# TopJohn/corda

Measured on AMD Instinct MI355X. Metric: signature verifications/sec (whole node, 1/2/4/8 GPU) + % integer-ALU peak, higher is better.
Workload: dtype u32

## Files before the change

### corda_amd/csrc/ed25519.hip

```cpp
#ifndef FE_QUAD
#define FE_QUAD 0
#endif
#ifndef FE_USE_ASM2
#define FE_USE_ASM2 1
#endif
#include <hip/hip_runtime.h>

#include <functional>
#include <stdint.h>
#include <stdlib.h>

#include "ed25519_ops.hpp"
#include "ed25519_route.hpp"
#include "ed25519_ws.hpp"
#include "sha2_device.hpp"
#include "status.hpp"

namespace cordahip {

__global__ void __launch_bounds__(64) ed25519_btable_kernel(uint32_t* __restrict__ tab) {
  const int g = blockIdx.x * blockDim.x + threadIdx.x;
  if (g >= 2 * kBTableEntries) return;
  const int k = g % kBTableEntries;
  ge_p3 B, P;
  ge_base(B);
  if (g >= kBTableEntries)
    for (int t = 0; t < kBDigits * kBBits; t++) ge_dbl<true>(B, B);
  ge_cached bc;
  ge_to_cached(bc, B);
  ge_identity(P);
  for (int bit = kBBits - 1; bit >= 0; bit--) {
    ge_dbl<true>(P, P);
    if ((k >> bit) & 1) ge_add<true>(P, P, bc);
  }
  store_niels_entry(tab + g * kBEntryWords, P);
  if (g == 0) {
    ge_cached id;
    fe_set(id.YpX, 1);
    fe_set(id.YmX, 1);
    fe_set(id.Z, 1);
    fe_set(id.T2d, 0);
    store_cached(tab + kBIdentityWord, id);
  }
}

CDEV bool mp8_ge(const uint32_t a[8], const uint32_t b[8]) {
  uint32_t br = 0;
#pragma unroll
  for (int i = 0; i < 8; i++) br = (uint32_t)(((uint64_t)a[i] - b[i] - br) >> 63);
  return br == 0;
}
CDEV void mp8_add(uint32_t r[8], const uint32_t a[8], const uint32_t b[8]) {
  uint64_t c = 0;
#pragma unroll
  for (int i = 0; i < 8; i++) {
    c += (uint64_t)a[i] + b[i];
    r[i] = (uint32_t)c;
    c >>= 32;
  }
}
CDEV void mp8_neg(uint32_t a[8]) {
  uint64_t c = 1;
#pragma unroll
  for (int i = 0; i < 8; i++) {
    c += (uint64_t)(~a[i]);
    a[i] = (uint32_t)c;
    c >>= 32;
  }
}
CDEV void mp8_copy(uint32_t d[8], const uint32_t s[8]) {
#pragma unroll
  for (int i = 0; i < 8; i++) d[i] = s[i];
}
CDEV int mp8_absbits(const uint32_t a[8]) {
  uint32_t t[8];
  mp8_copy(t, a);
  if (a[7] >> 31) mp8_neg(t);
  return mp8_bitlen(t);
}

CDEV double mp8_f64(const uint32_t a[8]) {
  double d = (double)a[7];
#pragma unroll
  for (int i = 6; i >= 0; i--) d = fma(d, 4294967296.0, (double)a[i]);
  return d;
}
CDEV void mp8_submul(uint32_t a[8], const uint32_t b[8], uint32_t q) {
  uint64_t pc = 0;
  uint32_t br = 0;
#pragma unroll
  for (int i = 0; i < 8; i++) {
    const uint64_t p = (uint64_t)q * b[i] + pc;
    pc = p >> 32;
    const uint64_t d = (uint64_t)a[i] - (uint32_t)p - br;
    a[i] = (uint32_t)d;
    br = (uint32_t)(d >> 63);
  }
}
CDEV void mp8_shl_dyn(uint32_t o[8], const uint32_t b[8], int k) {
  const int ws = k >> 5, bs = k & 31;
#pragma unroll
  for (int i = 0; i < 8; i++) {
    const uint32_t lo = (i - ws >= 0) ? word_sel(b, i - ws) : 0u;
    const uint32_t lo2 = (i - ws - 1 >= 0) ? word_sel(b, i - ws - 1) : 0u;
    o[i] = bs ? ((lo << bs) | (lo2 >> (32 - bs))) : lo;
  }
}

CDEV void euclid_divstep(uint32_t rp[8], const uint32_t rc[8], uint32_t tp[8], const uint32_t tc[8]) {
  const double inv = 1.0 / mp8_f64(rc);
  while (mp8_ge(rp, rc)) {
    const double qd = mp8_f64(rp) * inv * (1.0 - 0x1p-40);
    if (qd < 4294967296.0) {
      uint32_t q = (uint32_t)qd;
      q = q ? q : 1u;
      mp8_submul(rp, rc, q);
      mp8_submul(tp, tc, q);
    } else {
      const int e = (int)((__double_as_longlong(qd) >> 52) & 0x7ff) - 1023;
      const int k = e - 31;
      const uint32_t q = (uint32_t)(qd * __longlong_as_double((long long)(1023 - k) << 52));
      uint32_t bs[8], ts[8];
      mp8_shl_dyn(bs, rc, k);
      mp8_shl_dyn(ts, tc, k);
      mp8_submul(rp, bs, q);
      mp8_submul(tp, ts, q);
    }
  }
}

CDEV double mp8_top(const uint32_t a[8], int s) {
  const int w = s >> 5, b = s & 31;
  const uint64_t lo = ((uint64_t)word_sel(a, w + 1) << 32) | word_sel(a, w);
  const uint64_t hi = word_sel(a, w + 2);
  return (double)((lo >> b) | (b ? hi << (64 - b) : 0ull));
}
CDEV void mp8_lincomb(uint32_t o[8], const uint32_t x[8], int a, const uint32_t y[8], int b) {
  const uint32_t ua = (uint32_t)(a < 0 ? -a : a), ub = (uint32_t)(b < 0 ? -b : b);
  uint64_t pc = 0, qc = 0;
  uint32_t br = 0;
#pragma unroll
  for (int i = 0; i < 8; i++) {
    const uint64_t p = (uint64_t)ua * x[i] + pc;
    pc = p >> 32;
    const uint64_t q = (uint64_t)ub * y[i] + qc;
    qc = q >> 32;
    const uint64_t d = (uint64_t)(uint32_t)p - (uint32_t)q - br;
    o[i] = (uint32_t)d;
    br = (uint32_t)(d >> 63);
  }
  if (b > 0 || (b == 0 && a < 0)) mp8_neg(o);
}

CDEV void half_scalars(uint32_t c0abs[8], bool& c0neg, uint32_t c1[8], const uint32_t h[8]) {
  const uint32_t kM[8] = {0xe7ae9f68u, 0xc09318d2u, 0x17bce6b2u, 0xa6f7cef5u, 0u, 0u, 0u, 0x80000000u};
  const uint32_t kS[8] = {0x754abea0u, 0x597d89b3u, 0xf9de6484u, 0xb504f333u, 0u, 0u, 0u, 0u};
  uint32_t rp[8], rc[8], tp[8], tc[8];
#pragma unroll
  for (int i = 0; i < 8; i++) {
    rp[i] = kM[i];
    rc[i] = h[i];
    tp[i] = 0;
    tc[i] = i == 0;
  }
  for (;;) {
    const int s = max(mp8_bitlen(rp) - 52, 0);
    double uh = mp8_top(rp, s), vh = mp8_top(rc, s);
    const double th = mp8_top(kS, s) + 1.0;
    double A = 1.0, B = 0.0, C = 0.0, D = 1.0;
    int n = 0;
    for (;;) {
      const double d1 = vh + C, d2 = vh + D;
      if (!(d1 > 0.0 && d2 > 0.0)) break;
      const double n1 = uh + A;
      double q = floor(n1 / d1);
      const double r1 = fma(-q, d1, n1);
      q = r1 < 0.0 ? q - 1.0 : (r1 >= d1 ? q + 1.0 : q);
      const double r2 = fma(-q, d2, uh + B);
      if (!(r2 >= 0.0 && r2 < d2)) break;
      const double nC = fma(-q, C, A), nD = fma(-q, D, B), nv = fma(-q, vh, uh);
      const double mc = fmax(fabs(nC), fabs(nD));
      if (nv - mc < th || mc >= 0x1p30) break;
      A = C;
      B = D;
      C = nC;
      D = nD;
      uh = vh;
      vh = nv;
      n++;
    }
    if (n == 0) break;
    const int a = (int)A, b = (int)B, c = (int)C, d = (int)D;
    uint32_t x[8], y[8];
    mp8_lincomb(x, rp, a, rc, b);
    mp8_lincomb(y, rp, c, rc, d);
    mp8_copy(rp, x);
    mp8_copy(rc, y);
    mp8_lincomb(x, tp, a, tc, b);
    mp8_lincomb(y, tp, c, tc, d);
    mp8_copy(tp, x);
    mp8_copy(tc, y);
  }
  while (mp8_ge(rc, kS)) {
    euclid_divstep(rp, rc, tp, tc);
#pragma unroll
    for (int i = 0; i < 8; i++) {
      const uint32_t a = rp[i], b = tp[i];
      rp[i] = rc[i];
      rc[i] = a;
      tp[i] = tc[i];
      tc[i] = b;
    }
  }
  uint32_t a0[8], a1[8];
  mp8_copy(a0, rc);
  mp8_copy(a1, tc);
  if (!(tc[0] & 1)) {
    uint32_t r3[8], t3[8];
    mp8_copy(r3, rp);
    mp8_copy(t3, tp);
    euclid_divstep(r3, rc, t3, tc);
    uint32_t p0[8], p1[8], m0[8], m1[8], nr3[8], nt3[8];
    mp8_add(p0, rc, r3);
    mp8_add(p1, tc, t3);
    mp8_copy(nr3, r3);
    mp8_neg(nr3);
    mp8_copy(nt3, t3);
    mp8_neg(nt3);
    mp8_add(m0, rc, nr3);
    mp8_add(m1, tc, nt3);
    int best = max(mp8_absbits(r3), mp8_absbits(t3));
    mp8_copy(a0, r3);
    mp8_copy(a1, t3);
    const int bp = max(mp8_absbits(p0), mp8_absbits(p1));
    if (bp < best) {
      best = bp;
      mp8_copy(a0, p0);
      mp8_copy(a1, p1);
    }
    const int bm = max(mp8_absbits(m0), mp8_absbits(m1));
    if (bm < best) {
      mp8_copy(a0, m0);
      mp8_copy(a1, m1);
    }
  }
  if (a1[7] >> 31) {
    mp8_neg(a0);
    mp8_neg(a1);
  }
  c0neg = (a0[7] >> 31) != 0;
  if (c0neg) mp8_neg(a0);
  mp8_copy(c0abs, a0);
  mp8_copy(c1, a1);
}

CDEV bool ge_strict_ok(const ge_p3& R, const uint32_t w[8]) {
  uint32_t all_ones = (w[7] & 0x7fffffffu) == 0x7fffffffu;
#pragma unroll
  for (int i = 1; i < 7; i++) all_ones &= (w[i] == 0xffffffffu);
  if (all_ones && w[0] >= 0xffffffedu) return false;
  return !((w[7] >> 31) && fe_iszero(R.X));
}

CDEV void store_point(uint32_t* __restrict__ o, const ge_p3& p) {
  uint4* o4 = reinterpret_cast<uint4*>(o);
  uint32_t w[32];
#pragma unroll
  for (int i = 0; i < 10; i++) {
    w[i] = p.X.v[i];
    w[10 + i] = p.Y.v[i];
    w[20 + i] = p.T.v[i];
  }
  w[30] = w[31] = 0;
#pragma unroll
  for (int q = 0; q < 8; q++) o4[q] = make_uint4(w[4 * q], w[4 * q + 1], w[4 * q + 2], w[4 * q + 3]);
}
CDEV void load_point(ge_p3& p, const uint32_t* __restrict__ o) {
  const uint4* o4 = reinterpret_cast<const uint4*>(o);
  uint32_t w[32];
#pragma unroll
  for (int q = 0; q < 8; q++) {
    const uint4 v = o4[q];
    w[4 * q] = v.x;
    w[4 * q + 1] = v.y;
    w[4 * q + 2] = v.z;
    w[4 * q + 3] = v.w;
  }
#pragma unroll
  for (int i = 0; i < 10; i++) {
    p.X.v[i] = w[i];
    p.Y.v[i] = w[10 + i];
    p.T.v[i] = w[20 + i];
  }
  fe_set(p.Z, 1);
}

#ifndef ED_PREP_LDS
#define ED_PREP_LDS 1
#endif
#if !ED_PREP_LDS
static constexpr int kParkP = joint_index(2, 2), kParkQ = joint_index(2, -2);
#endif
static constexpr int kPqT2d = 30, kPqQ = 40, kPqWords = 70;

CDEV uint32_t* joint_slot(uint32_t* rec, int idx) { return rec + kWhTab + idx * kWhEntryWords; }

CDEV void pq_store(uint32_t* col, int at, const fe& f) {
#pragma unroll
  for (int i = 0; i < 10; i++) col[(at + i) * 256] = f.v[i];
}
CDEV void pq_load(fe& f, const uint32_t* col, int at) {
#pragma unroll
  for (int i = 0; i < 10; i++) f.v[i] = col[(at + i) * 256];
}

CDEV void load_cached_niels(ge_niels& n, const uint32_t* __restrict__ p) {
  ge_cached c;
  load_cached(c, p);
  n.ypx = c.YpX;
  n.ymx = c.YmX;
  n.xy2d = c.T2d;
}

CDEV void park_point(uint32_t* __restrict__ rec, uint32_t* col, int which, const ge_p3& p) {
#if ED_PREP_LDS
  pq_store(col, which * kPqQ, p.X);
  pq_store(col, which * kPqQ + 10, p.Y);
  pq_store(col, which * kPqQ + 20, p.T);
#else
  store_point(joint_slot(rec, which ? kParkQ : kParkP), p);
#endif
}
CDEV void load_parked(ge_p3& p, uint32_t* __restrict__ rec, const uint32_t* col, int which) {
#if ED_PREP_LDS
  pq_load(p.X, col, which * kPqQ);
  pq_load(p.Y, col, which * kPqQ + 10);
  pq_load(p.T, col, which * kPqQ + 20);
  fe_set(p.Z, 1);
#else
  load_point(p, joint_slot(rec, which ? kParkQ : kParkP));
#endif
}
CDEV void park_niels(uint32_t* col, int pass, const ge_cached& c) {
#if ED_PREP_LDS
  if (pass) {
    pq_store(col, kPqQ, c.YpX);
    pq_store(col, kPqQ + 10, c.YmX);
    pq_store(col, kPqQ + 20, c.T2d);
  } else {
    pq_store(col, kPqT2d, c.T2d);
  }
#endif
}
CDEV void load_parked_niels(ge_niels& n, uint32_t* __restrict__ rec, const uint32_t* col, int which) {
#if ED_PREP_LDS
  if (which) {
    pq_load(n.ypx, col, kPqQ);
    pq_load(n.ymx, col, kPqQ + 10);
    pq_load(n.xy2d, col, kPqQ + 20);
  } else {
    fe x, y;
    pq_load(x, col, 0);
    pq_load(y, col, 10);
    fe_add(n.ypx, y, x);
    fe_sub(n.ymx, y, x);
    pq_load(n.xy2d, col, kPqT2d);
  }
#else
  load_cached_niels(n, joint_slot(rec, which ? joint_index(0, 1) : joint_index(1, 0)));
#endif
}

CDEV void joint_single_pass(uint32_t* __restrict__ rec, uint32_t* col, int pass) {
  ge_p3 B, D;
  load_parked(B, rec, col, pass);
  ge_cached c;
  ge_to_cached(c, B);
  park_niels(col, pass, c);
  store_cached(joint_slot(rec, pass ? joint_index(0, 1) : joint_index(1, 0)), c);
  ge_dbl<true>(D, B);
  ge_to_cached(c, D);
  store_cached(joint_slot(rec, pass ? joint_index(0, 2) : joint_index(2, 0)), c);
}

CDEV void joint_sign_pass(uint32_t* __restrict__ rec, uint32_t* col, int s) {
  ge_p3 D, E;
  ge_niels nq, np;
  ge_cached c;
  load_parked(D, rec, col, 0);
  load_parked_niels(nq, rec, col, 1);
  niels_cneg(nq, s < 0);
  ge_madd<true>(D, D, nq);
  ge_to_cached(c, D);
  store_cached(joint_slot(rec, joint_index(1, s)), c);
  ge_madd<true>(E, D, nq);
  ge_to_cached(c, E);
  store_cached(joint_slot(rec, joint_index(1, 2 * s)), c);
#if ED_PREP_LDS
  PHASE_BARRIER();
#endif
  load_parked_niels(np, rec, col, 0);
  ge_madd<true>(E, D, np);
  ge_to_cached(c, E);
  store_cached(joint_slot(rec, joint_index(2, s)), c);
  ge_dbl<true>(E, D);
  ge_to_cached(c, E);
  store_cached(joint_slot(rec, joint_index(2, 2 * s)), c);
}


#ifndef ED_PREP_WAVES
#define ED_PREP_WAVES 2
#endif
CDEV uint8_t prep_decode_phase(const uint8_t* __restrict__ keys, const uint8_t* __restrict__ sigs, uint64_t i,
                               uint32_t msg_len, const uint8_t* __restrict__ pre_status, uint32_t empty_is_error,
                               uint32_t* __restrict__ rec, uint32_t* col, uint32_t abyte[8], uint32_t Rw[8]) {
  uint8_t st = kStatusPending;
  load8(Rw, reinterpret_cast<const uint32_t*>(sigs + i * 64));
  {
    uint32_t wa[8];
    load8(wa, reinterpret_cast<const uint32_t*>(keys + i * 32));
    ge_p3 A, R;
    bool okA, okR;
    ge_frombytes_i2p_pair(A, okA, wa, R, okR, Rw);
    if (!okA) st = kStatusBadKey;
    else if (pre_status && pre_status[i] != kStatusOk) st = pre_status[i];
    else if (msg_len == 0 && empty_is_error) st = kStatusEmpty;
    fe_tobytes(abyte, A.Y);
    abyte[7] |= fe_isnegative(A.X) << 31;
    if (st == kStatusPending && !(okR && ge_strict_ok(R, Rw))) st = kStatusBadSig;
    if (st != kStatusPending) {
      ge_identity(A);
      ge_identity(R);
    }
    fe_neg(A.X, A.X);
    fe_neg(A.T, A.T);
    fe_neg(R.X, R.X);
    fe_neg(R.T, R.T);
    park_point(rec, col, 0, A);
    park_point(rec, col, 1, R);
  }
  return st;
}

CDEV void prep_table_phase(uint32_t* __restrict__ rec, uint32_t* col) {
#pragma unroll 1
  for (int pass = 0; pass < 2; pass++) {
    joint_single_pass(rec, col, pass);
    PHASE_BARRIER();
  }
#pragma unroll 1
  for (int s = -1; s <= 1; s += 2) {
    joint_sign_pass(rec, col, s);
    PHASE_BARRIER();
  }
}

CDEV uint8_t prep_keys_phase(const uint8_t* __restrict__ keys, const uint8_t* __restrict__ sigs, uint64_t i,
                             uint32_t msg_len, const uint8_t* __restrict__ pre_status, uint32_t empty_is_error,
                             uint32_t* __restrict__ rec, uint32_t* col, uint32_t abyte[8], uint32_t Rw[8]) {
  const uint8_t st = prep_decode_phase(keys, sigs, i, msg_len, pre_status, empty_is_error, rec, col, abyte, Rw);
  PHASE_BARRIER();
  prep_table_phase(rec, col);
  return st;
}

CDEV void prep_msg_phase(const uint8_t* __restrict__ sigs, const uint8_t* __restrict__ msgs, uint32_t msg_len,
                         uint64_t i, uint8_t st, const uint32_t abyte[8], const uint32_t Rw[8],
                         uint32_t* __restrict__ rec) {
  uint32_t ka[8], kr[8], e[8];
  bool c0neg = false;
  if (st == kStatusPending) {
    uint32_t S[8], hd[16], h[8], se[8], zero[8];
    load8(S, reinterpret_cast<const uint32_t*>(sigs + i * 64 + 32));
    sha512_segments(hd, Rw, abyte, true, msgs + i * (uint64_t)msg_len, msg_len);
    sc_reduce512(h, hd);
    sc_effective_S(se, S, slide_drops_carry(S));
    half_scalars(ka, c0neg, kr, h);
#pragma unroll
    for (int q = 0; q < 8; q++) zero[q] = 0;
    sc_muladd(e, kr, se, zero);
  } else {
#pragma unroll
    for (int q = 0; q < 8; q++) ka[q] = kr[q] = e[q] = 0;
  }
#if ED_SEL_STREAM
  uint32_t sel[32];
  sel_recode(sel, ka, kr, e, c0neg);
  sel[kSelWords] = 0;
  uint4* o4 = reinterpret_cast<uint4*>(rec + kWhSel);
#pragma unroll
  for (int q = 0; q < 8; q++) o4[q] = make_uint4(sel[4 * q], sel[4 * q + 1], sel[4 * q + 2], sel[4 * q + 3]);
#else
  store8(rec + kWhKa, ka);
  store8(rec + kWhKr, kr);
  store8(rec + kWhE, e);
  reinterpret_cast<uint4*>(rec + kWhFlags)[0] = make_uint4(c0neg ? 1u : 0u, 0u, 0u, 0u);
#endif
}

#if ED_PREP_LDS
#define PREP_PARK_COLUMN(col)                  \
  __shared__ uint32_t pq_lds[kPqWords][256]; \
  uint32_t* col = &pq_lds[0][threadIdx.x]
#else
#define PREP_PARK_COLUMN(col) uint32_t* col = nullptr
#endif

__global__ void __launch_bounds__(256) __attribute__((amdgpu_waves_per_eu(ED_PREP_WAVES))) ed25519_prep_half_kernel(
    const uint8_t* __restrict__ keys, const uint8_t* __restrict__ sigs, const uint8_t* __restrict__ msgs,
    uint32_t msg_len, uint64_t base, uint64_t m, const uint8_t* __restrict__ pre_status,
    uint8_t* __restrict__ status, uint32_t* __restrict__ ws, uint32_t empty_is_error) {
  const uint64_t li = (uint64_t)blockIdx.x * blockDim.x + threadIdx.x;
  if (li >= m) return;
  const uint64_t i = base + li;
  uint32_t* rec = ws + li * kWhLaneWords;
  uint32_t abyte[8], Rw[8];
  PREP_PARK_COLUMN(col);
  const uint8_t st = prep_keys_phase(keys, sigs, i, msg_len, pre_status, empty_is_error, rec, col, abyte, Rw);
  prep_msg_phase(sigs, msgs, msg_len, i, st, abyte, Rw, rec);
  status[i] = st;
}

__global__ void __launch_bounds__(256) __attribute__((amdgpu_waves_per_eu(ED_PREP_WAVES)))
ed25519_prep_half_idx_kernel(const uint8_t* __restrict__ keys, const uint8_t* __restrict__ sigs,
                             const uint8_t* __restrict__ msgs, uint32_t msg_len, uint64_t base, uint64_t m,
                             const uint8_t* __restrict__ pre_status, uint8_t* __restrict__ status,
                             uint32_t* __restrict__ ws, uint32_t empty_is_error, const uint32_t* __restrict__ scratch,
                             uint64_t lanes) {
  const uint64_t li = (uint64_t)blockIdx.x * blockDim.x + threadIdx.x;
  if (li >= route_chunk_lanes(scratch[kRouteCntGeneric], base, m)) return;
  const uint64_t i = scratch[route_off_generic(lanes) + base + li];
  uint32_t* rec = ws + li * kWhLaneWords;
  uint32_t abyte[8], Rw[8];
  PREP_PARK_COLUMN(col);
  const uint8_t st = prep_keys_phase(keys, sigs, i, msg_len, pre_status, empty_is_error, rec, col, abyte, Rw);
  prep_msg_phase(sigs, msgs, msg_len, i, st, abyte, Rw, rec);
  status[i] = st;
}

__global__ void __launch_bounds__(256) __attribute__((amdgpu_waves_per_eu(ED_PREP_WAVES))) ed25519_prep_keys_kernel(
    const uint8_t* __restrict__ keys, const uint8_t* __restrict__ sigs, uint32_t msg_len, uint64_t base, uint64_t m,
    const uint8_t* __restrict__ pre_status, uint8_t* __restrict__ status, uint32_t* __restrict__ ws,
    uint32_t empty_is_error) {
  const uint64_t li = (uint64_t)blockIdx.x * blockDim.x + threadIdx.x;
  if (li >= m) return;
  const uint64_t i = base + li;
  uint32_t* rec = ws + li * kWhLaneWords;
  uint32_t abyte[8], Rw[8];
  PREP_PARK_COLUMN(col);
  status[i] = prep_keys_phase(keys, sigs, i, msg_len, pre_status, empty_is_error, rec, col, abyte, Rw);
  store8(rec + kWhKa, abyte);
}

__global__ void __launch_bounds__(256) __attribute__((amdgpu_waves_per_eu(ED_PREP_WAVES))) ed25519_prep_msg_kernel(const uint8_t* __restrict__ sigs,
                                                               const uint8_t* __restrict__ msgs, uint32_t msg_len,
                                                               uint64_t base, uint64_t m,
                                                               const uint8_t* __restrict__ status,
                                                               uint32_t* __restrict__ ws) {
  const uint64_t li = (uint64_t)blockIdx.x * blockDim.x + threadIdx.x;
  if (li >= m) return;
  const uint64_t i = base + li;
  uint32_t* rec = ws + li * kWhLaneWords;
  uint32_t abyte[8], Rw[8];
  load8(abyte, rec + kWhKa);
  load8(Rw, reinterpret_cast<const uint32_t*>(sigs + i * 64));
  prep_msg_phase(sigs, msgs, msg_len, i, status[i], abyte, Rw, rec);
}

CDEV void fixed_base_mult(ge_p3& P, const uint32_t k[8], const uint32_t* __restrict__ btab) {
  ge_identity(P);
  for (int j = 31; j >= 0; j--) {
    if (j != 31) {
#pragma unroll
      for (int t = 0; t < 7; t++) ge_dbl<false>(P, P);
      ge_dbl<true>(P, P);
    }
    const int d = booth_digit<8>(k, j);
    ge_niels nb;
    load_niels(nb, btab, d < 0 ? -d : d);
    niels_cneg(nb, d < 0);
    ge_madd<true>(P, P, nb);
  }
}

__global__ void __launch_bounds__(256) ed25519_sign_kernel(const uint8_t* __restrict__ seeds,
                                                          const uint8_t* __restrict__ msgs, uint32_t msg_len,
                                                          uint64_t n, const uint32_t* __restrict__ btab,
                                                          uint8_t* __restrict__ pubs, uint8_t* __restrict__ sigs) {
  const uint64_t i = (uint64_t)blockIdx.x * blockDim.x + threadIdx.x;
  if (i >= n) return;
  uint32_t seed[8];
  {
    const uint4* s4 = reinterpret_cast<const uint4*>(seeds + i * 32);
    const uint4 a = s4[0], b = s4[1];
    seed[0] = a.x; seed[1] = a.y; seed[2] = a.z; seed[3] = a.w;
    seed[4] = b.x; seed[5] = b.y; seed[6] = b.z; seed[7] = b.w;
  }
  const uint8_t* msg = msgs + i * (uint64_t)msg_len;
  uint32_t hs[16], dummy[8];
#pragma unroll
  for (int q = 0; q < 8; q++) dummy[q] = 0;
  sha512_segments(hs, seed, dummy, false, msg, 0);
  uint32_t a[8], prefix[8];
#pragma unroll
  for (int q = 0; q < 8; q++) {
    a[q] = hs[q];
    prefix[q] = hs[8 + q];
  }
  a[0] &= ~7u;
  a[7] &= 0x3fffffffu;
  a[7] |= 0x40000000u;
  uint32_t a16[16], ar[8];
#pragma unroll
  for (int q = 0; q < 8; q++) {
    a16[q] = a[q];
    a16[8 + q] = 0;
  }
  sc_reduce512(ar, a16);
  ge_p3 A;
  fixed_base_mult(A, ar, btab);
  uint32_t pub[8];
  ge_tobytes(pub, A);
  uint32_t rh[16], r[8];
  sha512_segments(rh, prefix, dummy, false, msg, msg_len);
  sc_reduce512(r, rh);
  ge_p3 Rp;
  fixed_base_mult(Rp, r, btab);
  uint32_t R[8];
  ge_tobytes(R, Rp);
  uint32_t kh[16], k[8], S[8];
  sha512_segments(kh, R, pub, true, msg, msg_len);
  sc_reduce512(k, kh);
  sc_muladd(S, k, ar, r);
  uint4* p4 = reinterpret_cast<uint4*>(pubs + i * 32);
  p4[0] = make_uint4(pub[0], pub[1], pub[2], pub[3]);
  p4[1] = make_uint4(pub[4], pub[5], pub[6], pub[7]);
  uint4* s4 = reinterpret_cast<uint4*>(sigs + i * 64);
  s4[0] = make_uint4(R[0], R[1], R[2], R[3]);
  s4[1] = make_uint4(R[4], R[5], R[6], R[7]);
  s4[2] = make_uint4(S[0], S[1], S[2], S[3]);
  s4[3] = make_uint4(S[4], S[5], S[6], S[7]);
}

}

namespace cordahip {
hipError_t launch_ed25519_btable(uint32_t* tab, hipStream_t s) {
  hipLaunchKernelGGL(ed25519_btable_kernel, dim3((2 * kBTableEntries + 63) / 64), dim3(64), 0, s, tab);
  return hipGetLastError();
}
size_t ed25519_btable_bytes() { return ((size_t)kBIdentityWord + 64) * sizeof(uint32_t); }

size_t ed25519_ws_lane_bytes() { return kWhLaneWords * sizeof(uint32_t); }

hipError_t launch_ed25519_verify(const uint8_t* keys, const uint8_t* sigs, const uint8_t* msgs, uint32_t msg_len,
                                 uint64_t n, const uint32_t* btab, const uint8_t* pre_status, uint8_t* status,
                                 unsigned long long* verdict, uint32_t* ws, uint64_t ws_lanes, uint32_t flags,
                                 hipStream_t s, const std::function<hipError_t()>* before_msgs) {
  if (n == 0) return hipSuccess;
  if (!ws || ws_lanes < 64 || ws_lanes % 64) return hipErrorInvalidValue;
  bool msgs_ready = before_msgs == nullptr;
  for (uint64_t base = 0; base < n; base += ws_lanes) {
    const uint64_t m = n - base < ws_lanes ? n - base : ws_lanes;
    const uint32_t blocks = (uint32_t)((m + 255) / 256);
    hipError_t e = hipSuccess;
    if (msgs_ready) {
      hipLaunchKernelGGL(ed25519_prep_half_kernel, dim3(blocks), dim3(256), 0, s, keys, sigs, msgs, msg_len, base, m,
                         pre_status, status, ws, (flags & 1u) ? 0u : 1u);
      e = hipGetLastError();
    } else {
      hipLaunchKernelGGL(ed25519_prep_keys_kernel, dim3(blocks), dim3(256), 0, s, keys, sigs, msg_len, base, m,
                         pre_status, status, ws, (flags & 1u) ? 0u : 1u);
      e = hipGetLastError();
      e = e ? e : (*before_msgs)();
      msgs_ready = true;
      if (e == hipSuccess)
        hipLaunchKernelGGL(ed25519_prep_msg_kernel, dim3(blocks), dim3(256), 0, s, sigs, msgs, msg_len, base, m, status,
                           ws);
      e = e ? e : hipGetLastError();
    }
    if (e == hipSuccess) e = launch_ed25519_ladder(base, m, btab, ws, status, verdict, s);
    if (e != hipSuccess) return e;
  }
  return hipSuccess;
}

hipError_t launch_ed25519_verify_idx(const uint8_t* keys, const uint8_t* sigs, const uint8_t* msgs, uint32_t msg_len,
                                     uint64_t n, const uint32_t* btab, const uint8_t* pre_status, uint8_t* status,
                                     uint32_t* ws, uint64_t ws_lanes, uint32_t flags, const uint32_t* scratch,
                                     hipStream_t s) {
  if (n == 0) return hipSuccess;
  if (!ws || ws_lanes < 64 || ws_lanes % 64 || !scratch) return hipErrorInvalidValue;
  for (uint64_t base = 0; base < n; base += ws_lanes) {
    const uint64_t m = n - base < ws_lanes ? n - base : ws_lanes;
    const uint32_t blocks = (uint32_t)((m + 255) / 256);
    hipLaunchKernelGGL(ed25519_prep_half_idx_kernel, dim3(blocks), dim3(256), 0, s, keys, sigs, msgs, msg_len, base, m,
                       pre_status, status, ws, (flags & 1u) ? 0u : 1u, scratch, n);
    hipError_t e = hipGetLastError();
    if (e == hipSuccess) e = launch_ed25519_ladder_idx(base, m, btab, ws, status, scratch, n, s);
    if (e != hipSuccess) return e;
  }
  return hipSuccess;
}

hipError_t launch_ed25519_sign(const uint8_t* seeds, const uint8_t* msgs, uint32_t msg_len, uint64_t n,
                               const uint32_t* btab, uint8_t* pubs, uint8_t* sigs, hipStream_t s) {
  if (n == 0) return hipSuccess;
  const uint64_t blocks = (n + 255) / 256;
  hipLaunchKernelGGL(ed25519_sign_kernel, dim3((uint32_t)blocks), dim3(256), 0, s, seeds, msgs, msg_len, n, btab,
                     pubs, sigs);
  return hipGetLastError();
}
}
```

### corda_amd/csrc/ed25519_ladder.hip

```cpp
#ifndef FE_USE_ASM2
#define FE_USE_ASM2 1
#endif
#include <hip/hip_runtime.h>
#include <stdint.h>

#include "ed25519_route.hpp"
#include "ed25519_ws.hpp"
#include "status.hpp"

namespace cordahip {

__device__ __attribute__((aligned(64))) const uint32_t kIdentityCached[kWhEntryWords] = {1, 0, 0, 0, 0, 0, 0, 0, 0, 0,
                                                            1, 0, 0, 0, 0, 0, 0, 0, 0, 0,
                                                            1, 0, 0, 0, 0, 0, 0, 0, 0, 0,
                                                            0, 0, 0, 0, 0, 0, 0, 0, 0, 0};

#ifndef ED_LADDER_WAVES
#define ED_LADDER_WAVES 2
#endif
static_assert(512 / ED_LADDER_WAVES >= 168, "fe25519_asm.hpp's v160..v167 accumulators need >= 168 VGPRs per lane");

template <bool kIdx>
CDEV void ladder_half_lane(uint64_t base, uint64_t m, const uint32_t* __restrict__ btab,
                           const uint32_t* __restrict__ ws, uint8_t* __restrict__ status,
                           unsigned long long* __restrict__ verdict, const uint32_t* __restrict__ list) {
  const uint64_t li = (uint64_t)blockIdx.x * blockDim.x + threadIdx.x;
  const bool active = li < m;
  const uint64_t lc = active ? li : m - 1;
  const uint32_t* rec = ws + lc * kWhLaneWords;
#if ED_IDENT_GLOBAL
  const uint32_t* ident = btab + kBIdentityWord;
#else
  const uint32_t* ident = kIdentityCached;
#endif
  const uint32_t* btab2 = btab + kBTableEntries * kBEntryWords;
  ge_p3 P;
  ge_identity(P);
#if ED_SEL_STREAM
  __shared__ uint32_t sk[kSelWords][256];
  {
    const uint4* r4 = reinterpret_cast<const uint4*>(rec + kWhSel);
#pragma unroll
    for (int q = 0; q < (kSelWords + 3) / 4; q++) {
      const uint4 v = r4[q];
      const uint32_t w[4] = {v.x, v.y, v.z, v.w};
#pragma unroll
      for (int t = 0; t < 4; t++)
        if (4 * q + t < kSelWords) sk[4 * q + t][threadIdx.x] = w[t];
    }
  }
  const uint32_t* col = &sk[0][threadIdx.x];
  const int W = min(max(wave_max((int)(col[kSelMeta * 256] >> 16)), (kBDigits - 1) * (kBBits / 2) + 1), kSelWindows);
  uint32_t selw = col[((W - 1) / kSelPerWord) * 256];
  for (int j = W - 1; j >= 0; j--) {
    const int jn = max(j - 1, 0);
    const uint32_t selw_next = col[(jn / kSelPerWord) * 256];
    const uint32_t sel = selw >> (kSelBits * (j % kSelPerWord));
    const uint32_t idx = sel & 15u;
    const bool neg = sel & kSelNeg;
    ge_cached c;
    load_cached(c, idx == kSelIdentity ? ident : rec + kWhTab + idx * kWhEntryWords);
    const bool bwin = j % (kBBits / 2) == 0 && j < kBDigits * (kBBits / 2);
    uint32_t m0 = 0, m1 = 0, sg = 0;
    const int t = j / (kBBits / 2);
    if (bwin) {
      m0 = col[(kSelMag + (t >> 1)) * 256];
      m1 = col[(kSelMag + ((t + kBDigits) >> 1)) * 256];
      sg = col[kSelMeta * 256];
    }
    if (j != W - 1) {
      ge_dbl<false>(P, P);
      ge_dbl<true>(P, P);
    }
    cached_cneg(c, neg);
    if (bwin) {
      const int sh = 16 * (t & 1);
      ge_niels nb0, nb1;
      uint32_t pad0[2], pad1[2];
      load_niels(nb0, btab, (int)((m0 >> sh) & 0xffffu), pad0);
      ge_add<true>(P, P, c);
      load_niels(nb1, btab2, (int)((m1 >> sh) & 0xffffu), pad1);
      niels_pad_use(pad0);
      niels_cneg(nb0, (sg >> t) & 1u);
      ge_madd<true>(P, P, nb0);
      niels_pad_use(pad1);
      niels_cneg(nb1, (sg >> (t + kBDigits)) & 1u);
      ge_madd<false>(P, P, nb1);
    } else {
      ge_add<false>(P, P, c);
    }
    selw = selw_next;
  }
#else
  __shared__ uint32_t sk[24][256];
  const uint32_t* ska = &sk[0][threadIdx.x];
  const uint32_t* skr = &sk[8][threadIdx.x];
  const uint32_t* ske = &sk[16][threadIdx.x];
  int bits;
  {
    uint32_t ka[8], kr[8], e[8];
    load8(ka, rec + kWhKa);
    load8(kr, rec + kWhKr);
    load8(e, rec + kWhE);
#pragma unroll
    for (int q = 0; q < 8; q++) {
      sk[q][threadIdx.x] = ka[q];
      sk[8 + q][threadIdx.x] = kr[q];
      sk[16 + q][threadIdx.x] = e[q];
    }
    bits = max(mp8_bitlen(ka), mp8_bitlen(kr));
  }
  const bool c0neg = rec[kWhFlags] & 1u;
  const int W = max(wave_max((bits + 2) / 2), (kBDigits - 1) * (kBBits / 2) + 1);
  for (int j = W - 1; j >= 0; j--) {
    const joint_sel sel = joint_select(joint_booth2(ska, 256, 8, j), joint_booth2(skr, 256, 8, j), c0neg);
    ge_cached c;
    load_cached(c, table_entry(rec, sel.idx, ident));
    if (j != W - 1) {
      ge_dbl<false>(P, P);
      ge_dbl<true>(P, P);
    }
    cached_cneg(c, sel.neg);
    const bool bwin = j % (kBBits / 2) == 0 && j < kBDigits * (kBBits / 2);
    if (bwin) {
      const int d0 = booth_digit_col<kBBits>(ske, j / (kBBits / 2));
      const int d1 = booth_digit_col<kBBits>(ske, j / (kBBits / 2) + kBDigits);
      ge_niels nb0, nb1;
      load_niels(nb0, btab, d0 < 0 ? -d0 : d0);
      ge_add<true>(P, P, c);
      load_niels(nb1, btab2, d1 < 0 ? -d1 : d1);
      niels_cneg(nb0, d0 < 0);
      ge_madd<true>(P, P, nb0);
      niels_cneg(nb1, d1 < 0);
      ge_madd<false>(P, P, nb1);
    } else {
      ge_add<false>(P, P, c);
    }
  }
#endif
  fe d;
  fe_sub(d, P.Y, P.Z);
  const bool zero = fe_iszero(P.X) && fe_iszero(d);
  const uint64_t i = kIdx ? (active ? list[base + li] : 0) : base + li;
  uint8_t st = kStatusBadSig;
  if (active) {
    st = status[i];
    if (st == kStatusPending) {
      st = zero ? kStatusOk : kStatusBadSig;
      status[i] = st;
    }
  }
  if (!kIdx) {
    const unsigned long long ok = __ballot(active && st == kStatusOk);
    if ((threadIdx.x & 63) == 0 && active && verdict) verdict[i >> 6] = ok;
  }
}

__global__ void __launch_bounds__(256) __attribute__((amdgpu_waves_per_eu(ED_LADDER_WAVES))) ed25519_ladder_half_kernel(
    uint64_t base, uint64_t m, const uint32_t* __restrict__ btab, const uint32_t* __restrict__ ws,
    uint8_t* __restrict__ status, unsigned long long* __restrict__ verdict) {
  ladder_half_lane<false>(base, m, btab, ws, status, verdict, nullptr);
}

__global__ void __launch_bounds__(256) __attribute__((amdgpu_waves_per_eu(ED_LADDER_WAVES)))
ed25519_ladder_half_idx_kernel(uint64_t base, uint64_t m, const uint32_t* __restrict__ btab,
                               const uint32_t* __restrict__ ws, uint8_t* __restrict__ status,
                               const uint32_t* __restrict__ scratch, uint64_t lanes) {
  const uint64_t mm = route_chunk_lanes(scratch[kRouteCntGeneric], base, m);
  if ((uint64_t)blockIdx.x * blockDim.x >= mm) return;
  ladder_half_lane<true>(base, mm, btab, ws, status, nullptr, scratch + route_off_generic(lanes));
}

hipError_t launch_ed25519_ladder(uint64_t base, uint64_t m, const uint32_t* btab, const uint32_t* ws, uint8_t* status,
                                 unsigned long long* verdict, hipStream_t s) {
  const uint32_t blocks = (uint32_t)((m + 255) / 256);
  hipLaunchKernelGGL(ed25519_ladder_half_kernel, dim3(blocks), dim3(256), 0, s, base, m, btab, ws, status, verdict);
  return hipGetLastError();
}

hipError_t launch_ed25519_ladder_idx(uint64_t base, uint64_t m, const uint32_t* btab, const uint32_t* ws,
                                     uint8_t* status, const uint32_t* scratch, uint64_t lanes, hipStream_t s) {
  const uint32_t blocks = (uint32_t)((m + 255) / 256);
  hipLaunchKernelGGL(ed25519_ladder_half_idx_kernel, dim3(blocks), dim3(256), 0, s, base, m, btab, ws, status, scratch,
                     lanes);
  return hipGetLastError();
}

}
```

Measured before the change: 108.4 million.

## Sort ladder lanes by window count within block and widen half-scalar candidate search

Each 256-thread block now ranks its lanes by the per-lane selector window count, using ballot and popcount plus a shared-memory prefix. Lanes with similar loop lengths then share a wave, which cuts the wave_max-driven wasted iterations. Verdict bitmasks are rebuilt in the original lane order by the last wave to finish, through a workgroup atomic counter. Separately, the scalar half-size decomposition is moved to a header and now considers six candidate pairs filtered to odd c1, aiming for shorter scalars at the cost of extra setup, a shared-memory sort, barriers and added complexity.

```diff
diff --git a/corda_amd/csrc/ed25519.hip b/corda_amd/csrc/ed25519.hip
--- a/corda_amd/csrc/ed25519.hip
+++ b/corda_amd/csrc/ed25519.hip
@@ -10,6 +10,7 @@
 #include <stdint.h>
 #include <stdlib.h>
 
+#include "ed25519_half.hpp"
 #include "ed25519_ops.hpp"
 #include "ed25519_route.hpp"
 #include "ed25519_ws.hpp"
@@ -44,90 +45,6 @@
   }
 }
 
-CDEV bool mp8_ge(const uint32_t a[8], const uint32_t b[8]) {
-  uint32_t br = 0;
-#pragma unroll
-  for (int i = 0; i < 8; i++) br = (uint32_t)(((uint64_t)a[i] - b[i] - br) >> 63);
-  return br == 0;
-}
-CDEV void mp8_add(uint32_t r[8], const uint32_t a[8], const uint32_t b[8]) {
-  uint64_t c = 0;
-#pragma unroll
-  for (int i = 0; i < 8; i++) {
-    c += (uint64_t)a[i] + b[i];
-    r[i] = (uint32_t)c;
-    c >>= 32;
-  }
-}
-CDEV void mp8_neg(uint32_t a[8]) {
-  uint64_t c = 1;
-#pragma unroll
-  for (int i = 0; i < 8; i++) {
-    c += (uint64_t)(~a[i]);
-    a[i] = (uint32_t)c;
-    c >>= 32;
-  }
-}
-CDEV void mp8_copy(uint32_t d[8], const uint32_t s[8]) {
-#pragma unroll
-  for (int i = 0; i < 8; i++) d[i] = s[i];
-}
-CDEV int mp8_absbits(const uint32_t a[8]) {
-  uint32_t t[8];
-  mp8_copy(t, a);
-  if (a[7] >> 31) mp8_neg(t);
-  return mp8_bitlen(t);
-}
-
-CDEV double mp8_f64(const uint32_t a[8]) {
-  double d = (double)a[7];
-#pragma unroll
-  for (int i = 6; i >= 0; i--) d = fma(d, 4294967296.0, (double)a[i]);
-  return d;
-}
-CDEV void mp8_submul(uint32_t a[8], const uint32_t b[8], uint32_t q) {
-  uint64_t pc = 0;
-  uint32_t br = 0;
-#pragma unroll
-  for (int i = 0; i < 8; i++) {
-    const uint64_t p = (uint64_t)q * b[i] + pc;
-    pc = p >> 32;
-    const uint64_t d = (uint64_t)a[i] - (uint32_t)p - br;
-    a[i] = (uint32_t)d;
-    br = (uint32_t)(d >> 63);
-  }
-}
-CDEV void mp8_shl_dyn(uint32_t o[8], const uint32_t b[8], int k) {
-  const int ws = k >> 5, bs = k & 31;
-#pragma unroll
-  for (int i = 0; i < 8; i++) {
-    const uint32_t lo = (i - ws >= 0) ? word_sel(b, i - ws) : 0u;
-    const uint32_t lo2 = (i - ws - 1 >= 0) ? word_sel(b, i - ws - 1) : 0u;
-    o[i] = bs ? ((lo << bs) | (lo2 >> (32 - bs))) : lo;
-  }
-}
-
-CDEV void euclid_divstep(uint32_t rp[8], const uint32_t rc[8], uint32_t tp[8], const uint32_t tc[8]) {
-  const double inv = 1.0 / mp8_f64(rc);
-  while (mp8_ge(rp, rc)) {
-    const double qd = mp8_f64(rp) * inv * (1.0 - 0x1p-40);
-    if (qd < 4294967296.0) {
-      uint32_t q = (uint32_t)qd;
-      q = q ? q : 1u;
-      mp8_submul(rp, rc, q);
-      mp8_submul(tp, tc, q);
-    } else {
-      const int e = (int)((__double_as_longlong(qd) >> 52) & 0x7ff) - 1023;
-      const int k = e - 31;
-      const uint32_t q = (uint32_t)(qd * __longlong_as_double((long long)(1023 - k) << 52));
-      uint32_t bs[8], ts[8];
-      mp8_shl_dyn(bs, rc, k);
-      mp8_shl_dyn(ts, tc, k);
-      mp8_submul(rp, bs, q);
-      mp8_submul(tp, ts, q);
-    }
-  }
-}
 
 CDEV double mp8_top(const uint32_t a[8], int s) {
   const int w = s >> 5, b = s & 31;
@@ -212,46 +129,7 @@
       tc[i] = b;
     }
   }
-  uint32_t a0[8], a1[8];
-  mp8_copy(a0, rc);
-  mp8_copy(a1, tc);
-  if (!(tc[0] & 1)) {
-    uint32_t r3[8], t3[8];
-    mp8_copy(r3, rp);
-    mp8_copy(t3, tp);
-    euclid_divstep(r3, rc, t3, tc);
-    uint32_t p0[8], p1[8], m0[8], m1[8], nr3[8], nt3[8];
-    mp8_add(p0, rc, r3);
-    mp8_add(p1, tc, t3);
-    mp8_copy(nr3, r3);
-    mp8_neg(nr3);
-    mp8_copy(nt3, t3);
-    mp8_neg(nt3);
-    mp8_add(m0, rc, nr3);
-    mp8_add(m1, tc, nt3);
-    int best = max(mp8_absbits(r3), mp8_absbits(t3));
-    mp8_copy(a0, r3);
-    mp8_copy(a1, t3);
-    const int bp = max(mp8_absbits(p0), mp8_absbits(p1));
-    if (bp < best) {
-      best = bp;
-      mp8_copy(a0, p0);
-      mp8_copy(a1, p1);
-    }
-    const int bm = max(mp8_absbits(m0), mp8_absbits(m1));
-    if (bm < best) {
-      mp8_copy(a0, m0);
-      mp8_copy(a1, m1);
-    }
-  }
-  if (a1[7] >> 31) {
-    mp8_neg(a0);
-    mp8_neg(a1);
-  }
-  c0neg = (a0[7] >> 31) != 0;
-  if (c0neg) mp8_neg(a0);
-  mp8_copy(c0abs, a0);
-  mp8_copy(c1, a1);
+  half_choose(c0abs, c0neg, c1, rp, rc, tp, tc);
 }
 
 CDEV bool ge_strict_ok(const ge_p3& R, const uint32_t w[8]) {
diff --git a/corda_amd/csrc/ed25519_half.hpp b/corda_amd/csrc/ed25519_half.hpp
--- /dev/null
+++ b/corda_amd/csrc/ed25519_half.hpp
@@ -0,0 +1,171 @@
+#pragma once
+#include <math.h>
+#include <stdint.h>
+
+#include "sc25519.hpp"
+
+#ifndef ED_HALF_SIX
+#define ED_HALF_SIX 1
+#endif
+
+namespace cordahip {
+
+CDEV bool mp8_ge(const uint32_t a[8], const uint32_t b[8]) {
+  uint32_t br = 0;
+#pragma unroll
+  for (int i = 0; i < 8; i++) br = (uint32_t)(((uint64_t)a[i] - b[i] - br) >> 63);
+  return br == 0;
+}
+CDEV void mp8_add(uint32_t r[8], const uint32_t a[8], const uint32_t b[8]) {
+  uint64_t c = 0;
+#pragma unroll
+  for (int i = 0; i < 8; i++) {
+    c += (uint64_t)a[i] + b[i];
+    r[i] = (uint32_t)c;
+    c >>= 32;
+  }
+}
+CDEV void mp8_sub(uint32_t r[8], const uint32_t a[8], const uint32_t b[8]) {
+  uint32_t br = 0;
+#pragma unroll
+  for (int i = 0; i < 8; i++) {
+    const uint64_t d = (uint64_t)a[i] - b[i] - br;
+    r[i] = (uint32_t)d;
+    br = (uint32_t)(d >> 63);
+  }
+}
+CDEV void mp8_neg(uint32_t a[8]) {
+  uint64_t c = 1;
+#pragma unroll
+  for (int i = 0; i < 8; i++) {
+    c += (uint64_t)(~a[i]);
+    a[i] = (uint32_t)c;
+    c >>= 32;
+  }
+}
+CDEV void mp8_copy(uint32_t d[8], const uint32_t s[8]) {
+#pragma unroll
+  for (int i = 0; i < 8; i++) d[i] = s[i];
+}
+CDEV int mp8_bits(const uint32_t a[8]) {
+  int n = 0;
+#pragma unroll
+  for (int i = 0; i < 8; i++) n = a[i] ? 32 * i + 32 - __builtin_clz(a[i]) : n;
+  return n;
+}
+CDEV int mp8_absbits(const uint32_t a[8]) {
+  uint32_t t[8];
+  mp8_copy(t, a);
+  if (a[7] >> 31) mp8_neg(t);
+  return mp8_bits(t);
+}
+
+CDEV double mp8_f64(const uint32_t a[8]) {
+  double d = (double)a[7];
+#pragma unroll
+  for (int i = 6; i >= 0; i--) d = fma(d, 4294967296.0, (double)a[i]);
+  return d;
+}
+CDEV void mp8_submul(uint32_t a[8], const uint32_t b[8], uint32_t q) {
+  uint64_t pc = 0;
+  uint32_t br = 0;
+#pragma unroll
+  for (int i = 0; i < 8; i++) {
+    const uint64_t p = (uint64_t)q * b[i] + pc;
+    pc = p >> 32;
+    const uint64_t d = (uint64_t)a[i] - (uint32_t)p - br;
+    a[i] = (uint32_t)d;
+    br = (uint32_t)(d >> 63);
+  }
+}
+CDEV void mp8_shl_dyn(uint32_t o[8], const uint32_t b[8], int k) {
+  const int ws = k >> 5, bs = k & 31;
+#pragma unroll
+  for (int i = 0; i < 8; i++) {
+    const uint32_t lo = (i - ws >= 0) ? word_sel(b, i - ws) : 0u;
+    const uint32_t lo2 = (i - ws - 1 >= 0) ? word_sel(b, i - ws - 1) : 0u;
+    o[i] = bs ? ((lo << bs) | (lo2 >> (32 - bs))) : lo;
+  }
+}
+CDEV uint64_t f64_bits(double d) {
+  uint64_t u;
+  __builtin_memcpy(&u, &d, 8);
+  return u;
+}
+CDEV double f64_from_bits(uint64_t u) {
+  double d;
+  __builtin_memcpy(&d, &u, 8);
+  return d;
+}
+
+CDEV void euclid_divstep(uint32_t rp[8], const uint32_t rc[8], uint32_t tp[8], const uint32_t tc[8]) {
+  const double inv = 1.0 / mp8_f64(rc);
+  while (mp8_ge(rp, rc)) {
+    const double qd = mp8_f64(rp) * inv * (1.0 - 0x1p-40);
+    if (qd < 4294967296.0) {
+      uint32_t q = (uint32_t)qd;
+      q = q ? q : 1u;
+      mp8_submul(rp, rc, q);
+      mp8_submul(tp, tc, q);
+    } else {
+      const int e = (int)((f64_bits(qd) >> 52) & 0x7ff) - 1023;
+      const int k = e - 31;
+      const uint32_t q = (uint32_t)(qd * f64_from_bits((uint64_t)(1023 - k) << 52));
+      uint32_t bs[8], ts[8];
+      mp8_shl_dyn(bs, rc, k);
+      mp8_shl_dyn(ts, tc, k);
+      mp8_submul(rp, bs, q);
+      mp8_submul(tp, ts, q);
+    }
+  }
+}
+
+CDEV void half_consider(uint32_t a0[8], uint32_t a1[8], int& best, const uint32_t x0[8], const uint32_t x1[8]) {
+  const int b0 = mp8_absbits(x0), b1 = mp8_absbits(x1);
+  const int b = b0 > b1 ? b0 : b1;
+  if ((x1[0] & 1u) && b < best) {
+    best = b;
+    mp8_copy(a0, x0);
+    mp8_copy(a1, x1);
+  }
+}
+
+CDEV void half_choose(uint32_t c0abs[8], bool& c0neg, uint32_t c1[8], const uint32_t rp[8], const uint32_t rc[8],
+                      const uint32_t tp[8], const uint32_t tc[8]) {
+  uint32_t a0[8], a1[8];
+  mp8_copy(a0, rc);
+  mp8_copy(a1, tc);
+  if (!(tc[0] & 1u)) {
+    int best = 1 << 30;
+    uint32_t r3[8], t3[8], x0[8], x1[8];
+    mp8_copy(r3, rp);
+    mp8_copy(t3, tp);
+    euclid_divstep(r3, rc, t3, tc);
+    half_consider(a0, a1, best, r3, t3);
+    mp8_add(x0, rc, r3);
+    mp8_add(x1, tc, t3);
+    half_consider(a0, a1, best, x0, x1);
+    mp8_sub(x0, rc, r3);
+    mp8_sub(x1, tc, t3);
+    half_consider(a0, a1, best, x0, x1);
+#if ED_HALF_SIX
+    half_consider(a0, a1, best, rp, tp);
+    mp8_add(x0, rp, rc);
+    mp8_add(x1, tp, tc);
+    half_consider(a0, a1, best, x0, x1);
+    mp8_sub(x0, rp, rc);
+    mp8_sub(x1, tp, tc);
+    half_consider(a0, a1, best, x0, x1);
+#endif
+  }
+  if (a1[7] >> 31) {
+    mp8_neg(a0);
+    mp8_neg(a1);
+  }
+  c0neg = (a0[7] >> 31) != 0;
+  if (c0neg) mp8_neg(a0);
+  mp8_copy(c0abs, a0);
+  mp8_copy(c1, a1);
+}
+
+}
diff --git a/corda_amd/csrc/ed25519_ladder.hip b/corda_amd/csrc/ed25519_ladder.hip
--- a/corda_amd/csrc/ed25519_ladder.hip
+++ b/corda_amd/csrc/ed25519_ladder.hip
@@ -20,11 +20,69 @@
 #endif
 static_assert(512 / ED_LADDER_WAVES >= 168, "fe25519_asm.hpp's v160..v167 accumulators need >= 168 VGPRs per lane");
 
+#ifndef ED_LADDER_ORDER
+#define ED_LADDER_ORDER 1
+#endif
+#if ED_LADDER_ORDER && !ED_SEL_STREAM
+#error "ED_LADDER_ORDER ranks the lanes by the selector stream's window count"
+#endif
+static constexpr int kOrderLo = 60, kOrderHi = 74, kOrderKeys = kOrderHi - kOrderLo + 2;
+static_assert(kOrderKeys <= 64, "one lane of a wave per key");
+
 template <bool kIdx>
 CDEV void ladder_half_lane(uint64_t base, uint64_t m, const uint32_t* __restrict__ btab,
                            const uint32_t* __restrict__ ws, uint8_t* __restrict__ status,
                            unsigned long long* __restrict__ verdict, const uint32_t* __restrict__ list) {
-  const uint64_t li = (uint64_t)blockIdx.x * blockDim.x + threadIdx.x;
+  const uint64_t blk = (uint64_t)blockIdx.x * blockDim.x;
+#if ED_LADDER_ORDER
+  __shared__ uint32_t sk[kSelWords][256];
+  __shared__ uint8_t order_src[256];
+  __shared__ uint32_t order_cnt[4][kOrderKeys];
+  __shared__ uint32_t order_done;
+  uint64_t li;
+  {
+    const uint64_t l0 = blk + threadIdx.x;
+    const uint32_t* r0 = ws + (l0 < m ? l0 : m - 1) * kWhLaneWords;
+    const uint4* r4 = reinterpret_cast<const uint4*>(r0 + kWhSel);
+    uint4 v[(kSelWords + 3) / 4];
+#pragma unroll
+    for (int q = 0; q < (kSelWords + 3) / 4; q++) v[q] = r4[q];
+    static_assert(kSelMeta == 30 && (kSelWords + 3) / 4 == 8, "the count is in the last quad's third word");
+    const int cnt = (int)(v[7].z >> 16);
+    const int key = l0 < m ? min(max(cnt, kOrderLo), kOrderHi) - kOrderLo : kOrderKeys - 1;
+    const int lane = threadIdx.x & 63, wave = threadIdx.x >> 6;
+    uint32_t before = 0, mine = 0;
+#pragma unroll
+    for (int k = 0; k < kOrderKeys; k++) {
+      const unsigned long long mk = __ballot(key == k);
+      if (key == k) before = (uint32_t)__popcll(mk & ((1ull << lane) - 1));
+      if (lane == k) mine = (uint32_t)__popcll(mk);
+    }
+    if (lane < kOrderKeys) order_cnt[wave][lane] = mine;
+    if (threadIdx.x == 0) order_done = 0;
+    __syncthreads();
+    uint32_t rank = before;
+#pragma unroll
+    for (int k = 0; k < kOrderKeys; k++)
+#pragma unroll
+      for (int w = 0; w < 4; w++) {
+        const uint32_t c = order_cnt[w][k];
+        rank += (k < key || (k == key && w < wave)) ? c : 0u;
+      }
+    order_src[rank] = (uint8_t)threadIdx.x;
+#pragma unroll
+    for (int q = 0; q < (kSelWords + 3) / 4; q++) {
+      const uint32_t w[4] = {v[q].x, v[q].y, v[q].z, v[q].w};
+#pragma unroll
+      for (int t = 0; t < 4; t++)
+        if (4 * q + t < kSelWords) sk[4 * q + t][rank] = w[t];
+    }
+    __syncthreads();
+    li = blk + order_src[threadIdx.x];
+  }
+#else
+  const uint64_t li = blk + threadIdx.x;
+#endif
   const bool active = li < m;
   const uint64_t lc = active ? li : m - 1;
   const uint32_t* rec = ws + lc * kWhLaneWords;
@@ -37,6 +95,7 @@
   ge_p3 P;
   ge_identity(P);
 #if ED_SEL_STREAM
+#if !ED_LADDER_ORDER
   __shared__ uint32_t sk[kSelWords][256];
   {
     const uint4* r4 = reinterpret_cast<const uint4*>(rec + kWhSel);
@@ -49,8 +108,14 @@
         if (4 * q + t < kSelWords) sk[4 * q + t][threadIdx.x] = w[t];
     }
   }
+#endif
   const uint32_t* col = &sk[0][threadIdx.x];
-  const int W = min(max(wave_max((int)(col[kSelMeta * 256] >> 16)), (kBDigits - 1) * (kBBits / 2) + 1), kSelWindows);
+#if ED_LADDER_ORDER
+  const int own = active ? (int)(col[kSelMeta * 256] >> 16) : 0;
+#else
+  const int own = (int)(col[kSelMeta * 256] >> 16);
+#endif
+  const int W = min(max(wave_max(own), (kBDigits - 1) * (kBBits / 2) + 1), kSelWindows);
   uint32_t selw = col[((W - 1) / kSelPerWord) * 256];
   for (int j = W - 1; j >= 0; j--) {
     const int jn = max(j - 1, 0);
@@ -151,8 +216,27 @@
     }
   }
   if (!kIdx) {
+#if ED_LADDER_ORDER
+    __shared__ uint8_t order_ok[256];
+    order_ok[li - blk] = active && st == kStatusOk;
+    __builtin_amdgcn_fence(__ATOMIC_RELEASE, "workgroup");
+    uint32_t arrived = 0;
+    if ((threadIdx.x & 63) == 0)
+      arrived = __hip_atomic_fetch_add(&order_done, 1u, __ATOMIC_RELAXED, __HIP_MEMORY_SCOPE_WORKGROUP);
+    arrived = (uint32_t)__shfl((int)arrived, 0);
+    if (arrived == blockDim.x / 64 - 1) {
+      __builtin_amdgcn_fence(__ATOMIC_ACQUIRE, "workgroup");
+      const int lane = threadIdx.x & 63;
+#pragma unroll
+      for (int q = 0; q < 4; q++) {
+        const unsigned long long ok = __ballot(order_ok[64 * q + lane] != 0);
+        if (lane == q && blk + 64 * q < m && verdict) verdict[(base + blk + 64 * q) >> 6] = ok;
+      }
+    }
+#else
     const unsigned long long ok = __ballot(active && st == kStatusOk);
     if ((threadIdx.x & 63) == 0 && active && verdict) verdict[i >> 6] = ok;
+#endif
   }
 }
 
```

Result: faster. 110.3 million, median of 6 (+1.8%).
